# mit-han-lab/llm-awq

Hardware: AMD Instinct MI355X
Metric: W4A16 decode+prefill tok/s, Llama-3-8B; achieved %HBM (GEMV) / %MFMA (GEMM) (higher is better)
Workload: dtype bf16; 1 GPU; Llama-3-8B W4A16 g128 bf16 activations on 1xMI355X (decode GEMV + prefill GEMM); layers=32, decode_m=1, prefill_m=2048, graph=True, layout=cdna4, clock_ramp_steps=60, decode_mlp=gate/up + SiLU*mul launch, then down_proj, prefill_mlp=SiLU*mul fused into the gate/up GEMM epilogue, mlp=interleaved, decode_side_buffer=sz_half, parallelism=tp1, full=False

## Files before the change

llm_awq_amd/csrc/awq_gemm_plan.hip:

```cpp
#include <string.h>

#include <type_traits>

#include "awq_device.hpp"
#include "awq_kernels.hpp"

namespace awq {

namespace {
constexpr int TM = 256;
constexpr double kNarrowRate = 0.80;
int g_small_m = 1;
int g_splitk = 1;
int g_v6 = 1;
int g_tile_n = 0;
int g_v6_192 = 1;
int g_v6_pair = 1;
int g_v6_szh = 1;
int g_v4 = 1;
void launch_wide(const void* x, const void* qw, const void* szp, const void* bias, void* out, int m, int n, int k, int n_begin,
                 int n_end, int dtype, hipStream_t st, int bits, int epi, const void* szh = nullptr, int tile_n = 256) {
  if (g_v6 && m >= 256) {
    if (szh != nullptr && bits == 4 && g_v6_szh) launch_gemm_cdna4_v6(x, qw, szh, bias, out, m, n, k, n_begin, n_end, dtype, st, bits, epi, 1, tile_n);
    else launch_gemm_cdna4_v6(x, qw, szp, bias, out, m, n, k, n_begin, n_end, dtype, st, bits, epi, 0, tile_n);
    return;
  }
  launch_gemm_cdna4_v4n(x, qw, szp, bias, out, m, n, k, n_begin, n_end, dtype, nullptr, 0, st, bits, epi);
}
int g_v6_128 = 1;
int narrow_kernel(int m, int n_cols, int k, int bits, bool has_ws, int epi) {
  const size_t wsb = g_splitk && has_ws && epi == 0 ? gemm_v4n_workspace_bytes(m, n_cols, k) : 0;
  if (wsb > 0) return (int)(wsb / ((size_t)((m + TM - 1) / TM) * ((n_cols + 127) / 128) * TM * 128 * 4));
  return g_v6_128 && g_v6 && bits == 4 && m >= TM ? 1 : 0;
}
void launch_narrow(const void* x, const void* qw, const void* szp, const void* bias, void* out, int m, int n, int k, int n_begin,
                   int n_end, int dtype, void* ws, size_t ws_bytes, hipStream_t st, int bits, int epi, const void* szh = nullptr) {
  const bool use_szh = szh != nullptr && bits == 4 && g_v6_szh;
  if (g_v6 && g_v6_pair && g_splitk && !g_tile_n && ws != nullptr && m >= TM &&
      launch_gemm_cdna4_v6_pair(x, qw, use_szh ? szh : szp, bias, out, m, n, k, n_begin, n_end, dtype, ws, ws_bytes, st, bits, epi, use_szh ? 1 : 0) == 0)
    return;
  if (narrow_kernel(m, n_end - n_begin, k, bits, ws != nullptr, epi) == 1) {
    launch_gemm_cdna4_v6(x, qw, use_szh ? szh : szp, bias, out, m, n, k, n_begin, n_end, dtype, st, bits, epi, use_szh ? 1 : 0, 128);
    return;
  }
  launch_gemm_cdna4_v4n(x, qw, szp, bias, out, m, n, k, n_begin, n_end, dtype, g_splitk ? ws : nullptr, ws_bytes, st, bits, epi);
}
}

namespace {
int g_moe_v4 = 1;
}
bool moe_v4_enabled() { return g_moe_v4 != 0; }
namespace {
int g_moe_v6 = 1;
}
bool moe_v6_enabled() { return g_moe_v6 != 0; }

int gemm_v3_tune_set(const char* key, int value) {
  if (!strcmp(key, "moe_v6")) g_moe_v6 = value;
  else if (!strcmp(key, "moe_tail")) moe_v6_set_tail(value);
  else if (!strcmp(key, "gemm_v4")) g_v4 = value;
  else if (!strcmp(key, "gemm_v6")) {
    g_v6 = value % 10;
    gemm_v6_set_probe(value / 10);
  }
  else if (!strcmp(key, "gemm_tile_n")) g_tile_n = value;
  else if (!strcmp(key, "gemm_v6_szh")) g_v6_szh = value;
  else if (!strcmp(key, "gemm_v6_pair")) g_v6_pair = value;
  else if (!strcmp(key, "gemm_v6_pair_lead")) gemm_v6_set_pair_lead(value);
  else if (!strcmp(key, "gemm_v6_pair_min_nit")) gemm_v6_set_pair_min_nit(value);
  else if (!strcmp(key, "gemm_v6_192")) g_v6_192 = value;
  else if (!strcmp(key, "gemm_v6_128")) g_v6_128 = value;
  else if (!strcmp(key, "moe_v4")) g_moe_v4 = value;
  else if (!strcmp(key, "gemm_small_m")) g_small_m = value;
  else if (!strcmp(key, "gemm_splitk_cap")) g_v4n_ksplit_cap = value;
  else if (!strcmp(key, "gemm_splitk")) {
    g_splitk = value;
    g_v4n_ksplit_force = value > 1 ? value : 0;
  }
  else return -1;
  return 0;
}

namespace {
struct Plan {
  int mode;
  long cols_main;
};
constexpr double k192Rate = 0.97;
Plan plan_tiles(int m, int n, int tile_n, bool allow192 = false) {
  if (tile_n == 128) return {1, 0};
  if (tile_n == 256) return {0, 0};
  if (tile_n == 192) return {allow192 ? 3 : 0, 0};
  const long tiles_m = (m + TM - 1) / TM;
  auto rounds = [](long t) { return (double)((t + 255) / 256); };
  const long cols256 = (n + 255) / 256, t256 = tiles_m * cols256;
  const double cost_wide = rounds(t256);
  const double cost_narrow = rounds(tiles_m * ((n + 127) / 128)) * 0.5 / kNarrowRate;
  const long cols_main = (t256 / 256) * 256 / tiles_m;
  double cost_mixed = 1e30;
  if (cols_main > 0 && cols_main < cols256) {
    const long n_rest = n - cols_main * 256;
    cost_mixed = rounds(tiles_m * cols_main) + rounds(tiles_m * ((n_rest + 127) / 128)) * 0.5 / kNarrowRate + 0.02;
  }
  const double cost_192 = allow192 ? rounds(tiles_m * ((n + 191) / 192)) * 0.75 / k192Rate : 1e30;
  if (cost_192 < cost_wide && cost_192 < cost_narrow && cost_192 < cost_mixed) return {3, 0};
  if (cost_mixed < cost_wide && cost_mixed < cost_narrow) return {2, cols_main};
  return {cost_narrow < cost_wide ? 1 : 0, 0};
}
}

bool gemm_cdna4_v3_takes(int m, int k) {
  if (m >= TM) return true;
  if (g_small_m == 2) return g_v4 && m > 8;
  return g_small_m && g_v4 && m >= 72 && (long)m * k >= 600000;
}

size_t gemm_cdna4_v3_workspace_bytes(int m, int n, int k) {
  if (!gemm_cdna4_v3_takes(m, k) || (n % 16) != 0 || (k % 128) != 0 || !g_v4 || !g_splitk) return 0;
  if (gemm_cdna4_v3_pair_plan(m, n, k)) return gemm_v6_pair_workspace_bytes(m, n, k);
  if (m < TM) return gemm_v4n_workspace_bytes(m, n, k);
  const Plan p = plan_tiles(m, n, 0);
  if (p.mode == 1) return gemm_v4n_workspace_bytes(m, n, k);
  if (p.mode == 2) {
    const int rest = n - (int)(p.cols_main * 256);
    return gemm_cdna4_v3_pair_plan(m, rest, k) ? gemm_v6_pair_workspace_bytes(m, rest, k) : gemm_v4n_workspace_bytes(m, rest, k);
  }
  return 0;
}

int gemm_cdna4_v3_pair_plan(int m, int n, int k) { return g_v6 && g_v6_pair && g_splitk && !g_tile_n && gemm_v6_pair_takes(m, n, k) ? 1 : 0; }

size_t gemm_cdna4_v3_workspace_bytes_w3(int m, int n, int k) {
  if (m <= 8 || (n % 16) != 0 || (k % 128) != 0 || !g_splitk) return 0;
  if (gemm_cdna4_v3_pair_plan(m, n, k)) return gemm_v6_pair_workspace_bytes(m, n, k);
  if (m < TM) return gemm_v4n_workspace_bytes(m, n, k);
  const Plan p = plan_tiles(m, n, 0);
  if (p.mode == 1) return gemm_v4n_workspace_bytes(m, n, k);
  if (p.mode == 2) {
    const int rest = n - (int)(p.cols_main * 256);
    return gemm_cdna4_v3_pair_plan(m, rest, k) ? gemm_v6_pair_workspace_bytes(m, rest, k) : gemm_v4n_workspace_bytes(m, rest, k);
  }
  return 0;
}

int gemm_cdna4_v3_plan(int m, int n, int bits, int* mode, int* cols_main) {
  if (m <= 8 || (n % 16) != 0) return 0;
  const bool allow192 = g_v6 != 0 && g_v6_192 != 0 && bits == 4 && m >= TM;
  const Plan p = m < TM ? Plan{1, 0} : plan_tiles(m, n, g_tile_n, allow192);
  if (mode) *mode = p.mode;
  if (cols_main) *cols_main = (int)p.cols_main;
  const long tm = (m + TM - 1) / TM;
  if (p.mode == 0) return (int)(tm * ((n + 255) / 256));
  if (p.mode == 1) return (int)(tm * ((n + 127) / 128));
  if (p.mode == 3) return (int)(tm * ((n + 191) / 192));
  return (int)(tm * p.cols_main + tm * ((n - p.cols_main * 256 + 127) / 128));
}

// ... 30 lines not shown
```

llm_awq_amd/csrc/awq_gemm_v4n.hip:

```cpp
#include <type_traits>

#include "awq_device.hpp"
#include "awq_kernels.hpp"

namespace awq {

namespace {
constexpr int TM = 256, TN = 128, TK = 64;
constexpr int kTileX = TM * TK * 2;
constexpr int kTileW = TN * TK * 2;
constexpr int kWBase = 2 * kTileX;
constexpr int WN = 32;
typedef float f32x16 __attribute__((ext_vector_type(16)));

__device__ __forceinline__ int swz(int row) { return (row & 7) ^ ((row >> 4) & 1); }
__device__ __forceinline__ int tile_off(int row, int gc) { return row * 128 + ((gc ^ swz(row)) << 4); }

struct Group {
  u32x4 w;
  u32 b01, b23;
  float c;
};
struct Raw {
  u32x4 w;
  u32 sz;
};
template <int V>
using ic = std::integral_constant<int, V>;
template <bool V>
using bc = std::integral_constant<bool, V>;
template <int WIDX, int ST>
struct JobT {
  static constexpr bool has = true;
  static constexpr int widx = WIDX, st = ST;
};
struct NoJob {
  static constexpr bool has = false;
  static constexpr int widx = 0, st = 0;
};
}

#define V4N_READ(dst, addr, off) asm volatile("ds_read_b128 %0, %1 offset:%2" : "=v"(dst) : "v"(addr), "n"(off) : "memory")
#define V4N_WRITE(addr, val, off) asm volatile("ds_write_b128 %0, %1 offset:%2\n\ts_nop 1" : : "v"(addr), "v"(val), "n"(off) : "memory")
#define V4N_FENCE() __builtin_amdgcn_sched_barrier(0)

template <typename DT, int KSPLIT, int PARTIAL, int BITS = 4>
__global__ __launch_bounds__(512) void gemm_cdna4_v4n_kernel(const uint16_t* __restrict__ x, const u32* __restrict__ qw,
                                                             const u32* __restrict__ szp, const uint16_t* __restrict__ bias,
                                                             uint16_t* __restrict__ out, int M, int N, int K, int tiles_m,
                                                             int tiles_n, int n_begin, int n_end, int ksplit,
                                                             float* __restrict__ partial, int epi) {
  using vec8 = typename DT::vec8;
  constexpr int kEpiRow = 2 * WN + 16;
  extern __shared__ __attribute__((aligned(16))) char smem[];
  const int tid = threadIdx.x, lane = tid & 63, wv = tid >> 6;
  const int i = lane & 15, g = lane >> 4;
  const int l32 = lane & 31, hk = lane >> 5;
  const int wm = wv >> 2, wn = wv & 3;

  const int T = tiles_m * tiles_n;
  const int split = KSPLIT ? (int)(blockIdx.x % (unsigned)ksplit) : 0;
  int tile;
  {
    const int b = KSPLIT ? (int)(blockIdx.x / (unsigned)ksplit) : (int)blockIdx.x, xcd = b & 7, idx = b >> 3;
    const int q = T >> 3, r = T & 7;
    tile = (xcd < r ? xcd * (q + 1) : r * (q + 1) + (xcd - r) * q) + idx;
  }
  int tm, tn;
  {
    const int full = (tiles_m >> 1) * 2 * tiles_n;
    if (tile < full) {
      const int band = tile / (2 * tiles_n), rem = tile - band * 2 * tiles_n;
      tn = rem >> 1;
      tm = 2 * band + (rem & 1);
    } else {
      tn = tile - full;
      tm = tiles_m - 1;
    }
  }
  const int m0 = max(min(tm * TM, M - TM), 0), n0 = n_begin + tn * TN;
  const int nit_all = K >> 7;
  const int g0 = KSPLIT ? split * nit_all / ksplit : 0;
  const int nit = KSPLIT ? (split + 1) * nit_all / ksplit - g0 : nit_all;

  u32 a_off[4];
  {
    const int row = tid >> 3, gcp = tid & 7;
    const int gc = gcp ^ swz(row);
#pragma unroll
    for (int q = 0; q < 4; ++q) a_off[q] = (u32)min(m0 + row + 64 * q, M - 1) * (u32)K + gc * 8;
  }
  const int a_rows = PARTIAL ? M - m0 - (tid >> 3) : 256;
  auto issue_a = [&](int kt, int stage) {
    char* dst = smem + stage * kTileX + wv * 1024;
#pragma unroll
    for (int q = 0; q < 4; ++q) {
      const uint16_t* xq = x + (size_t)(kt + 2 * g0) * TK;
      if (!PARTIAL || 64 * q < a_rows)
        __builtin_amdgcn_global_load_lds((const __attribute__((address_space(1))) void*)(xq + a_off[q]),
                                       (__attribute__((address_space(3))) void*)(dst + q * 8192), 16, 0, 0);
    }
  };

  const int nslab = N >> 4;
  const int sl = min((n0 >> 4) + wv, min(nslab, n_end >> 4) - 1);
  constexpr int kTileWords = BITS == 4 ? 256 : 192, kLaneWords = BITS == 4 ? 4 : 3;
  const u32 b_off = (u32)sl * nit_all * kTileWords + lane * kLaneWords, sz_off = (u32)sl * nit_all * 16 + i;
  const int nl = 16 * wv + i;
  Cdna4DequantT<DT> cd;
  cd.init(lane, BITS == 4 ? 0x000F000Fu : 0x00070007u);
  auto load_group = [&](int grp) {
    Raw r;
    const u32* wp = qw + (size_t)(g0 + grp) * kTileWords + b_off;
    if (BITS == 4) {
      r.w = *reinterpret_cast<const u32x4*>(wp);
    } else {
      typedef u32 u32x3 __attribute__((ext_vector_type(3)));
      const u32x3 w3 = *reinterpret_cast<const u32x3*>(wp);
      r.w = u32x4{w3.x, w3.y, w3.z, 0u};
    }
    r.sz = szp[(size_t)(g0 + grp) * 16 + sz_off];
    return r;
  };
  auto prep = [&](const Raw& r) {
    Group gq;
    gq.w = BITS == 4 ? r.w : w3_expand(r.w.x, r.w.y, r.w.z);
    const u32 sd = (r.sz & 0xFFFFu) * 0x00010001u;
    gq.b01 = sd & cd.m01;
    gq.b23 = sd & cd.m23;
    gq.c = DT::dq_offset(r.sz);
    return gq;
  };

  const u32 lds0 = (u32)(size_t)(__attribute__((address_space(3))) char*)smem;
// ... 64 lines not shown
      asm volatile("s_waitcnt lgkmcnt(3)" : "+v"(wc), "+v"(x0));
      mfb(ic<0>{}, wc, x0);
      V4N_FENCE();
      asm volatile("s_waitcnt lgkmcnt(2)" : "+v"(x1));
      mfb(ic<1>{}, wc, x1);
      V4N_FENCE();
      asm volatile("s_waitcnt lgkmcnt(0)" : "+v"(x2), "+v"(x3));
      __syncthreads();
      V4N_FENCE();
      if constexpr (J::has) {
        const vec8 v = Cdna4DequantT<DT>::word_finish(pj);
        V4N_WRITE(ja[J::widx & 1], __builtin_bit_cast(u32x4, v), J::st * kTileW);
      }
      if constexpr (RD) {
        V4N_READ(wnx, wa[KN], SN * kTileW);
        V4N_READ(x0, xa[KN], SN * kTileX);
        V4N_READ(x1, xa[KN], SN * kTileX + 4096);
      }
      V4N_FENCE();
      mfb(ic<2>{}, wc, x2);
      V4N_FENCE();
      if constexpr (RD) V4N_READ(x2, xa[KN], SN * kTileX + 8192);
      mfb(ic<3>{}, wc, x3);
      V4N_FENCE();
      if constexpr (RD) V4N_READ(x3, xa[KN], SN * kTileX + 12288);
      V4N_FENCE();
    }
  };

  issue_a(0, 0);
  gc = prep(load_group(0));
  Raw rn = load_group(nit > 1 ? 1 : 0);
  {
    char* Bs = smem + kWBase;
    *reinterpret_cast<vec8*>(Bs + tile_off(nl, 0 + g)) = cd.word(gc.w.x, gc.b01, gc.b23, gc.c);
    *reinterpret_cast<vec8*>(Bs + tile_off(nl, 4 + g)) = cd.word(gc.w.y, gc.b01, gc.b23, gc.c);
  }
  __syncthreads();
  asm volatile("" : "+v"(rn.w), "+v"(rn.sz));
  issue_a(1, 1);
  V4N_FENCE();
  {
    const vec8 v = cd.word(gc.w.z, gc.b01, gc.b23, gc.c);
    V4N_WRITE(ja[0], __builtin_bit_cast(u32x4, v), kTileW);
  }
  V4N_READ(wf[0], wa[0], 0);
  V4N_READ(x0, xa[0], 0);
  V4N_READ(x1, xa[0], 4096);
  V4N_READ(x2, xa[0], 8192);
  V4N_READ(x3, xa[0], 12288);
  V4N_FENCE();

  auto group_iter = [&](int q, auto more_tag) {
    constexpr bool more = decltype(more_tag)::value;
    using Tt = bc<true>;
    using Ff = bc<false>;
    step(ic<0>{}, ic<0>{}, ic<1>{}, Tt{}, Ff{}, NoJob{});
    step(ic<1>{}, ic<0>{}, ic<2>{}, Tt{}, Ff{}, JobT<3, 1>{});
    step(ic<0>{}, ic<0>{}, ic<3>{}, Tt{}, Ff{}, NoJob{});
    if constexpr (more) {
      gc = prep(rn);
      step(ic<1>{}, ic<1>{}, ic<0>{}, Tt{}, Tt{}, JobT<0, 0>{});
      rn = load_group(min(q + 2, nit - 1));
      issue_a(2 * q + 2, 0);
      V4N_FENCE();
      step(ic<0>{}, ic<1>{}, ic<1>{}, Tt{}, Ff{}, NoJob{});
      step(ic<1>{}, ic<1>{}, ic<2>{}, Tt{}, Ff{}, JobT<1, 0>{});
      step(ic<0>{}, ic<1>{}, ic<3>{}, Tt{}, Ff{}, NoJob{});
      step(ic<1>{}, ic<0>{}, ic<0>{}, Tt{}, Tt{}, JobT<2, 1>{});
      issue_a(2 * q + 3, 1);
      V4N_FENCE();
    } else {
      step(ic<1>{}, ic<1>{}, ic<0>{}, Tt{}, Tt{}, NoJob{});
      step(ic<0>{}, ic<1>{}, ic<1>{}, Tt{}, Ff{}, NoJob{});
      step(ic<1>{}, ic<1>{}, ic<2>{}, Tt{}, Ff{}, NoJob{});
      step(ic<0>{}, ic<1>{}, ic<3>{}, Tt{}, Ff{}, NoJob{});
      step(ic<1>{}, ic<0>{}, ic<0>{}, Ff{}, Tt{}, NoJob{});
    }
  };
  for (int q = 0; q + 1 < nit; ++q) group_iter(q, std::true_type{});
  group_iter(nit - 1, std::false_type{});

  if constexpr (KSPLIT != 0) {
    float* base = partial + (((size_t)tile * ksplit + split) * 8 + wv) * (4 * 4 * 64 * 4);
#pragma unroll
    for (int b = 0; b < 4; ++b)
#pragma unroll
      for (int j = 0; j < 4; ++j)
        *reinterpret_cast<f32x4*>(base + ((b * 4 + j) * 64 + lane) * 4) =
            f32x4{acc[b][4 * j + 0], acc[b][4 * j + 1], acc[b][4 * j + 2], acc[b][4 * j + 3]};
    return;
  }
  if (epi == 3) {
    float* o32 = reinterpret_cast<float*>(out);
#pragma unroll
    for (int b = 0; b < 4; ++b) {
      const int m = m0 + wm * 128 + b * 32 + l32;
#pragma unroll
      for (int j = 0; j < 4; ++j) {
        const int nn = n0 + wn * WN + 8 * j + 4 * hk;
        if (nn < n_end && m < M)
          __builtin_nontemporal_store(f32x4{acc[b][4 * j + 0], acc[b][4 * j + 1], acc[b][4 * j + 2], acc[b][4 * j + 3]}, reinterpret_cast<f32x4*>(o32 + (size_t)m * N + nn));
      }
    }
    return;
  }
  __syncthreads();
  char* eb = smem + wv * (128 * kEpiRow);
#pragma unroll
  for (int b = 0; b < 4; ++b)
#pragma unroll
    for (int j = 0; j < 4; ++j) {
      u32x2 v;
      v.x = (u32)DT::from_float(acc[b][4 * j + 0]) | ((u32)DT::from_float(acc[b][4 * j + 1]) << 16);
      v.y = (u32)DT::from_float(acc[b][4 * j + 2]) | ((u32)DT::from_float(acc[b][4 * j + 3]) << 16);
      *reinterpret_cast<u32x2*>(eb + (b * 32 + l32) * kEpiRow + (8 * j + 4 * hk) * 2) = v;
    }
  __builtin_amdgcn_s_waitcnt(0xc07f);
  __builtin_amdgcn_wave_barrier();
  constexpr int GR = WN / 8, RP = 64 / GR;
#pragma unroll
  for (int ps = 0; ps < 128 / RP; ++ps) {
    const int row = ps * RP + lane / GR, gc2 = lane % GR;
    const int m = m0 + wm * 128 + row, nn = n0 + wn * WN + gc2 * 8;
    u32x4 v = *reinterpret_cast<const u32x4*>(eb + row * kEpiRow + gc2 * 16);
    if (epi == 2) {
      if ((gc2 & 1) == 0 && nn < n_end && m < M) {
        const u32x4 u = *reinterpret_cast<const u32x4*>(eb + row * kEpiRow + (gc2 + 1) * 16);
        __builtin_nontemporal_store(silu_mul_octet<DT>(v, u), reinterpret_cast<u32x4*>(out + (size_t)m * (N >> 1) + (nn >> 1)));
      }
      continue;
    }
    if (nn < n_end && m < M) {
      if (bias != nullptr) {
        const u32x4 bv = *reinterpret_cast<const u32x4*>(bias + nn);
        auto add2 = [](u32 a, u32 b) {
          const float lo = DT::to_float((uint16_t)(a & 0xFFFFu)) + DT::to_float((uint16_t)(b & 0xFFFFu));
          const float hi = DT::to_float((uint16_t)(a >> 16)) + DT::to_float((uint16_t)(b >> 16));
          return (u32)DT::from_float(lo) | ((u32)DT::from_float(hi) << 16);
        };
        v = u32x4{add2(v.x, bv.x), add2(v.y, bv.y), add2(v.z, bv.z), add2(v.w, bv.w)};
      }
      __builtin_nontemporal_store(v, reinterpret_cast<u32x4*>(out + (size_t)m * N + nn));
    }
  }
}

template <typename DT>
__global__ __launch_bounds__(256) void splitk_reduce_kernel(const float* __restrict__ partial, const uint16_t* __restrict__ bias,
                                                            uint16_t* __restrict__ out, int M, int N, int tiles_m, int tiles_n,
                                                            int n_begin, int n_end, int ksplit) {
  constexpr int kRow = 2 * WN + 16;
  __shared__ __attribute__((aligned(16))) char stage[4][32 * kRow];
  const int lane = threadIdx.x & 63, w = threadIdx.x >> 6;
  const int piece = blockIdx.x * 4 + w;
  const int b = piece & 3, wv = (piece >> 2) & 7, tile = piece >> 5;
  if (tile >= tiles_m * tiles_n) return;
  const int l32 = lane & 31, hk = lane >> 5, wm = wv >> 2, wn = wv & 3;
  int tm, tn;
  {
    const int full = (tiles_m >> 1) * 2 * tiles_n;
    if (tile < full) {
      const int band = tile / (2 * tiles_n), rem = tile - band * 2 * tiles_n;
      tn = rem >> 1;
      tm = 2 * band + (rem & 1);
    } else {
      tn = tile - full;
      tm = tiles_m - 1;
    }
  }
  constexpr size_t kWaveFloats = 4 * 4 * 64 * 4;
  const float* p = partial + (((size_t)tile * ksplit) * 8 + wv) * kWaveFloats + ((size_t)(b * 4) * 64 + lane) * 4;
  f32x4 acc[4];
#pragma unroll
  for (int j = 0; j < 4; ++j) acc[j] = f32x4{0.f, 0.f, 0.f, 0.f};
  for (int s2 = 0; s2 < ksplit; ++s2) {
    f32x4 v[4];
#pragma unroll
    for (int j = 0; j < 4; ++j) v[j] = *reinterpret_cast<const f32x4*>(p + (size_t)s2 * 8 * kWaveFloats + j * 256);
#pragma unroll
    for (int j = 0; j < 4; ++j) acc[j] += v[j];
  }
  char* eb = stage[w];
#pragma unroll
  for (int j = 0; j < 4; ++j) {
    u32x2 v;
    v.x = (u32)DT::from_float(acc[j][0]) | ((u32)DT::from_float(acc[j][1]) << 16);
    v.y = (u32)DT::from_float(acc[j][2]) | ((u32)DT::from_float(acc[j][3]) << 16);
    *reinterpret_cast<u32x2*>(eb + l32 * kRow + (8 * j + 4 * hk) * 2) = v;
  }
  __builtin_amdgcn_s_waitcnt(0xc07f);
  __builtin_amdgcn_wave_barrier();
  const int m_base = max(min(tm * TM, M - TM), 0) + wm * 128 + b * 32, n_base = n_begin + tn * TN + wn * WN;
#pragma unroll
  for (int ps = 0; ps < 2; ++ps) {
    const int row = ps * 16 + (lane >> 2), gc2 = lane & 3;
    const int nn = n_base + gc2 * 8;
    u32x4 v = *reinterpret_cast<const u32x4*>(eb + row * kRow + gc2 * 16);
    if (nn < n_end && m_base + row < M) {
      if (bias != nullptr) {
        const u32x4 bv = *reinterpret_cast<const u32x4*>(bias + nn);
        auto add2 = [](u32 a, u32 c) {
          const float lo = DT::to_float((uint16_t)(a & 0xFFFFu)) + DT::to_float((uint16_t)(c & 0xFFFFu));
          const float hi = DT::to_float((uint16_t)(a >> 16)) + DT::to_float((uint16_t)(c >> 16));
          return (u32)DT::from_float(lo) | ((u32)DT::from_float(hi) << 16);
        };
        v = u32x4{add2(v.x, bv.x), add2(v.y, bv.y), add2(v.z, bv.z), add2(v.w, bv.w)};
      }
      *reinterpret_cast<u32x4*>(out + (size_t)(m_base + row) * N + nn) = v;
    }
  }
}

int g_v4n_ksplit_cap = 1;
int g_v4n_ksplit_force = 0;
int gemm_v4n_ksplit(int m, int n_cols, int k) {
  const long tiles = (long)((m + TM - 1) / TM) * ((n_cols + TN - 1) / TN);
  const int nit = k / 128;
  if (g_v4n_ksplit_force > 1) return g_v4n_ksplit_force <= nit && tiles * g_v4n_ksplit_force <= 1024 ? g_v4n_ksplit_force : 1;
  auto rounds = [](long blocks) { return (double)((blocks + 255) / 256); };
  const double unsplit = rounds(tiles) * (nit + 2.0);
  double best_cost = 0.9 * unsplit;
  int best = 1;
  for (int d = 2; d <= 16 && nit / d >= 2; ++d) {
    if (g_v4n_ksplit_cap && tiles * d > 192 && tiles * d <= 256 && nit / d <= 8) continue;
    const double cost = rounds(tiles * d) * ((nit + d - 1) / d + 0.6) + 0.041 * (double)(tiles * d) + 1.3;
    if (cost < best_cost) {
      best_cost = cost;
      best = d;
    }
  }
  return best;
}
size_t gemm_v4n_workspace_bytes(int m, int n_cols, int k) {
  const int ks = gemm_v4n_ksplit(m, n_cols, k);
  if (ks <= 1) return 0;
  const size_t tiles = (size_t)((m + TM - 1) / TM) * ((n_cols + TN - 1) / TN);
  return tiles * ks * (size_t)TM * TN * 4;
}

void launch_gemm_cdna4_v4n(const void* x, const void* qw, const void* szp, const void* bias, void* out, int m, int n, int k,
                           int n_begin, int n_end, int dtype, void* ws, size_t ws_bytes, hipStream_t st, int bits, int epi) {
  constexpr int smem_main = 2 * kTileX + 2 * kTileW;
  constexpr int smem_epi = 8 * 128 * (2 * WN + 16);
  constexpr int smem = smem_main > smem_epi ? smem_main : smem_epi;
  const int tiles_m = (m + TM - 1) / TM, tiles_n = (n_end - n_begin + TN - 1) / TN;
  using Kern = void (*)(const uint16_t*, const u32*, const u32*, const uint16_t*, uint16_t*, int, int, int, int, int, int, int, int, float*, int);
  static const Kern kerns4[2][2][2] = {
      {{gemm_cdna4_v4n_kernel<F16, 0, 0>, gemm_cdna4_v4n_kernel<F16, 0, 1>}, {gemm_cdna4_v4n_kernel<F16, 1, 0>, gemm_cdna4_v4n_kernel<F16, 1, 1>}},
      {{gemm_cdna4_v4n_kernel<BF16, 0, 0>, gemm_cdna4_v4n_kernel<BF16, 0, 1>}, {gemm_cdna4_v4n_kernel<BF16, 1, 0>, gemm_cdna4_v4n_kernel<BF16, 1, 1>}}};
  static const Kern kerns3[2][2][2] = {
      {{gemm_cdna4_v4n_kernel<F16, 0, 0, 3>, gemm_cdna4_v4n_kernel<F16, 0, 1, 3>}, {gemm_cdna4_v4n_kernel<F16, 1, 0, 3>, gemm_cdna4_v4n_kernel<F16, 1, 1, 3>}},
      {{gemm_cdna4_v4n_kernel<BF16, 0, 0, 3>, gemm_cdna4_v4n_kernel<BF16, 0, 1, 3>}, {gemm_cdna4_v4n_kernel<BF16, 1, 0, 3>, gemm_cdna4_v4n_kernel<BF16, 1, 1, 3>}}};
  const Kern (*kerns)[2][2] = bits == 3 ? kerns3 : kerns4;
  static LdsOptIn optin[2][8];
  for (int a = 0; a < 8; ++a) optin[bits == 3][a].ensure(reinterpret_cast<const void*>(kerns[a >> 2][(a >> 1) & 1][a & 1]), smem);
  const int dt = dtype == 0 ? 0 : 1, partial = m <= TM - 32 ? 1 : 0;
  const int ks = gemm_v4n_ksplit(m, n_end - n_begin, k);
  const size_t need = ks > 1 ? (size_t)tiles_m * tiles_n * ks * TM * TN * 4 : 0;
  if (epi == 0 && ks > 1 && ws != nullptr && ws_bytes >= need && (reinterpret_cast<uintptr_t>(ws) & 15) == 0) {
    hipLaunchKernelGGL(kerns[dt][1][partial], dim3(tiles_m * tiles_n * ks), dim3(512), smem, st, (const uint16_t*)x, (const u32*)qw,
                       (const u32*)szp, (const uint16_t*)nullptr, (uint16_t*)out, m, n, k, tiles_m, tiles_n, n_begin, n_end, ks, (float*)ws, 0);
    auto red = dtype == 0 ? splitk_reduce_kernel<F16> : splitk_reduce_kernel<BF16>;
    hipLaunchKernelGGL(red, dim3((unsigned)(tiles_m * tiles_n * 8)), dim3(256), 0, st, (const float*)ws, (const uint16_t*)bias, (uint16_t*)out,
                       m, n, tiles_m, tiles_n, n_begin, n_end, ks);
    return;
  }
  hipLaunchKernelGGL(kerns[dt][0][partial], dim3(tiles_m * tiles_n), dim3(512), smem, st, (const uint16_t*)x, (const u32*)qw,
                     (const u32*)szp, (const uint16_t*)bias, (uint16_t*)out, m, n, k, tiles_m, tiles_n, n_begin, n_end, 1, (float*)nullptr, epi);
}

}
```

llm_awq_amd/csrc/awq_kernels.hpp:

```cpp
#pragma once
#include <hip/hip_runtime.h>
#include <stddef.h>
#include <stdint.h>

#include <atomic>

namespace awq {
struct LdsOptIn {
  std::atomic<uint64_t> done[4] = {};
  void ensure(const void* kern, int bytes = 160 * 1024) {
    int dev = 0;
    (void)hipGetDevice(&dev);
    const uint64_t bit = 1ull << (dev & 63);
    std::atomic<uint64_t>& w = done[(dev >> 6) & 3];
    if (w.load(std::memory_order_acquire) & bit) return;
    (void)hipFuncSetAttribute(kern, hipFuncAttributeMaxDynamicSharedMemorySize, bytes);
    w.fetch_or(bit, std::memory_order_release);
  }
};
inline int device_cu_count() {
  static std::atomic<int> cached[64] = {};
  int dev = 0;
  if (hipGetDevice(&dev) != hipSuccess) return 256;
  std::atomic<int>& c = cached[dev & 63];
  int v = c.load(std::memory_order_relaxed);
  if (v == 0) {
    if (hipDeviceGetAttribute(&v, hipDeviceAttributeMultiprocessorCount, dev) != hipSuccess || v <= 0) v = 256;
    c.store(v, std::memory_order_relaxed);
  }
  return v;
}
int launch_gemv(const void* x, const void* qw, const void* s, const void* z, const void* szp, void* out, int m, int n,
                int k, int dtype, int layout, hipStream_t st);
int launch_gemv_cdna4(const void* x, const void* qw, const void* szp, const void* bias, void* out, int m, int n, int k,
                      int epi, int bits, int dtype, hipStream_t st);
int launch_gemv_cdna4_norm(const void* x, const void* gamma, float eps, const void* qw, const void* szp, const void* bias, void* out,
                           int m, int n, int k, int epi, int dtype, hipStream_t st);
bool gemv_v2fast_enabled();
int launch_gemv_v2fast(const void* x, const void* qw, const void* s, const void* z, const void* bias, void* out, int m, int n, int k,
                       int gpad, int dtype, hipStream_t st);
int launch_skinny_v2(const void* x, const void* qw, const void* s, const void* z, const void* bias, void* out, int m, int n, int k,
                     int gpad, int dtype, hipStream_t st);
int launch_pack_w3(const void* q_u8, void* qw3, int n, int k, hipStream_t st);
int launch_unpack_w3(const void* qw3, void* out_u8, int n, int k, hipStream_t st);
int launch_dequant_w3(const void* qw3, const void* s, const void* z, void* out, int n, int k, int dtype, hipStream_t st);
int launch_expand_w3_to_cdna4(const void* qw3, void* qw4, int n, int k, hipStream_t st);
int gemv_cdna4_tune_set(const char* key, int value);
int launch_gemv_dma(const void* x, const void* qw, const void* szp, const void* bias, void* out, int m, int n, int k, int epi,
                    int dtype, int szfmt, hipStream_t st, int f32out = 0);
int gemv_dma_tune_set(const char* key, int value);
int launch_moe_gemv_cdna4(const void* x, const void* qw, const void* szp, const void* offsets, void* out, int total_rows,
                          int experts, int n, int k, int dtype, hipStream_t st);
int launch_moe_skinny_tail_cdna4(const void* x, const void* qw, const void* szp, const void* offsets, void* out, int experts, int n, int k,
                                 int dtype, hipStream_t st, int epi, int tail);
void moe_v6_set_tail(int v);
int launch_moe_skinny_cdna4(const void* x, const void* qw, const void* szp, const void* offsets, void* out, int total_rows,
                            int experts, int n, int k, int dtype, hipStream_t st);
int launch_pack_sz_cdna4(const void* s, const void* z, void* szp, int n, int k, hipStream_t st);
int launch_pack_szh_cdna4(const void* s, const void* z, void* szh, int* inexact, int n, int k, int dtype, hipStream_t st);
int launch_gemm(const void* x, const void* qw, const void* s, const void* z, const void* szp, void* out, int m, int n,
                int k, int dtype, int layout, void* ws, size_t ws_bytes, hipStream_t st);
int launch_repack_v2_cdna4(const void* src, void* dst, int n, int k, int to_cdna4, hipStream_t st);
int launch_unpack_cdna4(const void* qw, void* out_u8, int n, int k, hipStream_t st);
int launch_dequant_cdna4(const void* qw, const void* s, const void* z, void* out, int n, int k, int dtype, hipStream_t st);
size_t gemm_workspace_bytes(int m, int n, int k);
int launch_gemm_cdna4_v3(const void* x, const void* qw, const void* szp, const void* bias, void* out, int m, int n, int k,
                         int tile_n, int dtype, void* ws, size_t ws_bytes, hipStream_t st, int bits = 4, int epi = 0, const void* szh = nullptr);
int gemm_variant_get();
int launch_skinny_cdna4(const void* x, const void* qw, const void* szp, const void* bias, void* out, int m, int n, int k,
                        int dtype, hipStream_t st, int f32out = 0, void* ws = nullptr, size_t ws_bytes = 0);
int launch_skinny_w3(const void* x, const void* qw, const void* szp, const void* bias, void* out, int m, int n, int k, int epi, int dtype, hipStream_t st,
                     int f32out = 0);
int launch_skinny_gate_up(const void* x, const void* qw, const void* szp, void* out, int m, int n2, int k, int dtype, hipStream_t st);
int skinny_splitk_parts(int m, int n, int k);
size_t skinny_splitk_workspace_bytes(int m, int n, int k);
int skinny_tune_set(const char* key, int value);
int launch_midm_cdna4(const void* x, const void* qw, const void* szp, const void* bias, void* out, int m, int n, int k, int epi, int dtype, int szfmt,
                      int bits, int f32out, void* ws, size_t ws_bytes, hipStream_t st);
bool midm_takes(int m, int n, int k);
size_t midm_workspace_bytes(int m, int n, int k);
int midm_parts(int m, int n, int k);
int midm_tune_set(const char* key, int value);
int midm_init();
unsigned* splitk_ticket_words(hipStream_t st, int groups);
int launch_skinny_decode(const void* x, const void* qw, const void* szp, const void* bias, void* out, int m, int n, int k, int epi,
                         int dtype, int szfmt, hipStream_t st, int f32out = 0);
int launch_moe_gemm(const void* x, const void* qw, const void* s, const void* z, const void* offsets, void* out, int total_m,
                    int experts, int n, int k, int gpad, int dtype, int layout, hipStream_t st);
int gemv_tune_set(const char* key, int value);
int gemm_tune_set(const char* key, int value);
int gemm_v3_tune_set(const char* key, int value);
void launch_gemm_cdna4_v4n(const void* x, const void* qw, const void* szp, const void* bias, void* out, int m, int n, int k,
                           int n_begin, int n_end, int dtype, void* ws, size_t ws_bytes, hipStream_t st, int bits = 4, int epi = 0);
size_t gemm_v4n_workspace_bytes(int m, int n_cols, int k);
extern int g_v4n_ksplit_force;
extern int g_v4n_ksplit_cap;
bool gemm_cdna4_v3_takes(int m, int k);
size_t gemm_cdna4_v3_workspace_bytes(int m, int n, int k);
int gemm_cdna4_v3_plan(int m, int n, int bits, int* mode, int* cols_main);
int gemm_cdna4_v3_narrow_kernel(int m, int n_cols, int k, int bits, int has_workspace, int epi);
int gemv_dma_plan(int m, int n, int k, int epi, int* kernel);
size_t gemm_cdna4_v3_workspace_bytes_w3(int m, int n, int k);
bool moe_v4_enabled();
int launch_moe_gemm_cdna4_v6(const void* x, const void* qw, const void* szp, const void* offsets, void* out, int total, int experts,
                             int n, int k, int dtype, hipStream_t st, int epi = 0, const void* szh = nullptr);
int launch_silu_mul_interleaved(const void* in, void* out, int m, int n2, int dtype, hipStream_t st);
int launch_silu_mul(const void* gate, const void* up, void* out, size_t count, int dtype, hipStream_t st);
bool moe_v6_enabled();
void launch_gemm_cdna4_v6(const void* x, const void* qw, const void* szp, const void* bias, void* out, int m, int n, int k, int n_begin,
                          int n_end, int dtype, hipStream_t st, int bits = 4, int epi = 0, int szfmt = 0, int tile_n = 256);
void gemm_v6_set_probe(int v);
bool gemm_v6_pair_takes(int m, int n, int k);
int gemm_v6_pair_lost(unsigned* count);
int gemm_cdna4_v3_pair_plan(int m, int n, int k);
size_t gemm_v6_pair_workspace_bytes(int m, int n, int k);
int launch_gemm_cdna4_v6_pair(const void* x, const void* qw, const void* szp, const void* bias, void* out, int m, int n, int k, int n_begin, int n_end,
                              int dtype, void* ws, size_t ws_bytes, hipStream_t st, int bits = 4, int epi = 0, int szfmt = 0);
void gemm_v6_set_pair_lead(int v);
void gemm_v6_set_pair_min_nit(int v);
int launch_bias_add(void* out, const void* bias, int m, int n, int dtype, hipStream_t st);
int launch_round_bias_f32(const void* in_f32, const void* bias, void* out, int m, int n, int dtype, hipStream_t st);
int launch_rmsnorm(const void* x, const void* gamma, float eps, void* out, int m, int k, int dtype, hipStream_t st);
int attn_decode_plan(int batch, int nheads_kv, int head_dim, int timestep, int lmax, int* splits, int* chunk);
size_t attn_decode_workspace_bytes(int batch, int nheads, int nheads_kv, int head_dim, int timestep, int lmax);
int launch_attn_decode(const void* q, const void* k, const void* v, void* k_cache, void* v_cache, const int* lens, const float* alibi,
                       void* out, int B, int H, int Hkv, int Dh, int Lmax, long long q_bs, long long k_bs, long long v_bs, int timestep,
                       int rot, float rot_base, float rot_scale, int neox, int dtype, void* workspace, hipStream_t st);
int attn_prefill_plan(int batch, int nheads, int nheads_kv, int head_dim, int seqlen_q, int seqlen_k, int causal, int* q_tile_rows,
                      int* blocks);
int attn_prefill_tune_set(const char* key, int value);
int launch_attn_prefill(const void* q, const void* k, const void* v, void* out, int B, int Sq, int Sk, int H, int Hkv, int Dh, long long q_bs,
                        long long q_rs, long long k_bs, long long k_rs, long long v_bs, long long v_rs, float scale, int causal, int dtype,
                        hipStream_t st);
int launch_rope_with_pos(const void* in, const float* freqs, void* out, int n0, int n1, int h, int d, int d2, long long s0, long long s1,
                         long long sh, long long o0, long long o1, long long oh, int dtype, hipStream_t st);
int launch_rope_neox(const long long* positions, void* query, void* key, const void* cache, int tokens, int heads, int head_size, int rot_dim,
                     int max_pos, int dtype, hipStream_t st);
int w8a8_gemm_plan(int m, int n, int k, int* tile_m, int* tile_n);
int w8a8_tune_set(const char* key, int value);
int launch_w8a8_gemm(const void* x, const void* w, const void* wscales, const void* ascales, const void* bias, void* out, int m, int n, int k,
                     hipStream_t st);
int launch_quant_per_token(const void* x, void* out_i8, void* scale, int m, int k, int dtype, hipStream_t st);
int launch_gelu_quant_per_token(const void* x, void* out_i8, void* scale, void* tmp, int m, int k, hipStream_t st);
int launch_layernorm_quant(const void* x, const void* gamma, const void* beta, float eps, void* out_i8, void* scale, int m, int k,
                           int per_token, int dtype, hipStream_t st);
int launch_unpack_v2(const void* qw, void* out_u8, int n, int k, hipStream_t st);
int launch_dequant_v2(const void* qw, const void* s, const void* z, void* out, int n, int k, int dtype, hipStream_t st);
int launch_pack_v2(const void* q_u8, void* qw, int n, int k, hipStream_t st);
int launch_repack_v1_to_v2(const void* qw1, const void* s1, const void* qz1, void* qw2, void* s2, void* sz2, int n, int k,
                           int gpad, int dtype, hipStream_t st);
}
```

llm_awq_amd/csrc/awq_midm_cdna4.hip:

```cpp
#include <string.h>

#include <atomic>
#include <mutex>
#include <type_traits>

#include "awq_device.hpp"
#include "awq_dma.hpp"
#include "awq_kernels.hpp"

#ifdef AWQ_ENABLE_PROBES
__device__ unsigned long long g_midm_stamps[2048 * 8];
extern "C" __attribute__((visibility("default"))) int awq_dev_midm_stamps(void* host_dst, int blocks) {
  return (int)hipMemcpyFromSymbol(host_dst, HIP_SYMBOL(g_midm_stamps), (size_t)blocks * 64, 0, hipMemcpyDeviceToHost);
}
#define MIDM_STAMP(j)                                                                \
  if (threadIdx.x == 0 && blockIdx.y == 0 && blockIdx.x < 2048) {                    \
    g_midm_stamps[blockIdx.x * 8 + 2 * (j)] = __builtin_amdgcn_s_memrealtime();      \
    g_midm_stamps[blockIdx.x * 8 + 2 * (j) + 1] = __builtin_readcyclecounter();      \
  }
#else
#define MIDM_STAMP(j)
#endif

namespace awq {

namespace {
constexpr u32 kOob = 0x80000000u;
}

template <int C, int CB>
__device__ __forceinline__ void midm_read_x(u32x4 (&dst)[CB], u32 addr) {
  if constexpr (C < CB) {
    asm volatile("ds_read_b128 %0, %1 offset:%2" : "=v"(dst[C]) : "v"(addr), "n"(C * 4096) : "memory");
    midm_read_x<C + 1, CB>(dst, addr);
  }
}

template <int S>
__device__ __forceinline__ void midm_read_w(u32x4& w, u32& sz, u32 waddr, u32 saddr) {
  asm volatile("ds_read_b128 %0, %1 offset:%2" : "=v"(w) : "v"(waddr), "n"(S * 1280) : "memory");
  asm volatile("ds_read_b32 %0, %1 offset:%2" : "=v"(sz) : "v"(saddr), "n"(S * 1280) : "memory");
}

template <typename DT, int THREADS, int NSB>
__device__ __forceinline__ void midm_reduce_parts(char* smem, const float* __restrict__ parts, u32* __restrict__ tickets, const uint16_t* __restrict__ bias,
                                                  uint16_t* __restrict__ out, int M, int N, int KS, int nb, int epi, int f32out) {
  const int nslab = N >> 4;
  auto to_f = [](uint16_t b) { return DT::to_float(b); };
  asm volatile("s_waitcnt vmcnt(0)" : : : "memory");
  __syncthreads();
  u32* bc = reinterpret_cast<u32*>(smem);
  if (threadIdx.x == 0) bc[0] = __hip_atomic_fetch_add(tickets + nb, 1u, __ATOMIC_RELAXED, __HIP_MEMORY_SCOPE_AGENT);
  __syncthreads();
  if (bc[0] != (u32)(KS - 1)) return;
  if (threadIdx.x == 0) __hip_atomic_store(tickets + nb, 0u, __ATOMIC_RELAXED, __HIP_MEMORY_SCOPE_AGENT);
  const int col0 = nb * NSB * 16;
  auto sum_quad = [&](int m, int col) {
    f32x4 a = f32x4{0.f, 0.f, 0.f, 0.f};
    for (int p0 = 0; p0 < KS; p0 += 4) {
      f32x4 v[4];
#pragma unroll
      for (int j = 0; j < 4; ++j) {
        const float* src = parts + ((size_t)min(p0 + j, KS - 1) * M + m) * N + col;
        asm volatile("global_load_dwordx4 %0, %1, off sc1" : "=v"(v[j]) : "v"(src) : "memory");
      }
      asm volatile("s_waitcnt vmcnt(0)" : "+v"(v[0]), "+v"(v[1]), "+v"(v[2]), "+v"(v[3]) : : "memory");
#pragma unroll
      for (int j = 0; j < 4; ++j)
        if (p0 + j < KS) a += v[j];
    }
    return a;
  };
  if (epi == 2) {
    constexpr int QC = NSB * 2;
    for (int idx = threadIdx.x; idx < M * QC; idx += THREADS) {
      const int m = idx / QC, q = idx - m * QC, sl = q >> 1, h = q & 1;
      const int slab = nb * NSB + sl;
      if (slab >= nslab) continue;
      const f32x4 gt4 = sum_quad(m, col0 + sl * 16 + 4 * h), up4 = sum_quad(m, col0 + sl * 16 + 8 + 4 * h);
      uint16_t o[4];
#pragma unroll
      for (int r = 0; r < 4; ++r) {
        const float gt = to_f(DT::from_float(gt4[r])), u = to_f(DT::from_float(up4[r]));
        const float sl2 = to_f(DT::from_float(silu_f32(gt)));
        o[r] = DT::from_float(sl2 * u);
      }
      *reinterpret_cast<u32x2*>(out + (size_t)m * (N >> 1) + slab * 8 + 4 * h) = u32x2{(u32)o[0] | ((u32)o[1] << 16), (u32)o[2] | ((u32)o[3] << 16)};
// ... 230 lines not shown
              if (bias != nullptr) o[r] = DT::from_float(to_f(o[r]) + to_f(bias[nn + r]));
            }
            *reinterpret_cast<u32x2*>(out + (size_t)m * N + nn) = u32x2{(u32)o[0] | ((u32)o[1] << 16), (u32)o[2] | ((u32)o[3] << 16)};
          }
        }
      }
    }
#ifdef AWQ_ENABLE_PROBES
    asm volatile("s_waitcnt vmcnt(0)" ::: "memory");
#endif
    MIDM_STAMP(3)
    return;
  }

  {
    float* mine = parts + (size_t)p * M * N;
#pragma unroll
    for (int s = 0; s < NS; ++s) {
      const int slab = nb * NSB + wv * NS + s;
#pragma unroll
      for (int c = 0; c < CB; ++c) {
        const int m = 16 * c + i;
        if (slab < nslab && m < M) {
          float* dst = mine + (size_t)m * N + slab * 16 + 4 * g;
          asm volatile("global_store_dwordx4 %0, %1, off sc1\n\ts_nop 1" : : "v"(dst), "v"(acc[s][c]) : "memory");
        }
      }
    }
  }
  midm_reduce_parts<DT, 64 * WAVES, NSB>(smem, parts, tickets, bias, out, M, N, KS, nb, epi, f32out);
}

namespace {
constexpr int kStreamLanes = 64, kLaneWords = 1024;
constexpr int kCaptureWords = 1 << 20;
struct TicketPool {
  u32* base = nullptr;
  hipStream_t lane_stream[kStreamLanes] = {};
  bool lane_used[kStreamLanes] = {};
  int capture_next = 0;
};
std::mutex g_ticket_mu;
TicketPool g_pools[64];
}


unsigned* splitk_ticket_words(hipStream_t st, int groups) {
  int dev = 0;
  if (st == hipStreamPerThread) return nullptr;
  if (groups > kLaneWords || hipGetDevice(&dev) != hipSuccess || dev < 0 || dev >= 64) return nullptr;
  hipStreamCaptureStatus cs = hipStreamCaptureStatusNone;
  if (st != nullptr && hipStreamIsCapturing(st, &cs) != hipSuccess) return nullptr;
  const bool capturing = cs != hipStreamCaptureStatusNone;
  std::lock_guard<std::mutex> lock(g_ticket_mu);
  TicketPool& tp = g_pools[dev];
  if (tp.base == nullptr) {
    if (capturing) return nullptr;
    u32* fresh = nullptr;
    const size_t bytes = ((size_t)kStreamLanes * kLaneWords + kCaptureWords) * sizeof(u32);
    if (hipMalloc(reinterpret_cast<void**>(&fresh), bytes) != hipSuccess) return nullptr;
    if (hipMemset(fresh, 0, bytes) != hipSuccess || hipStreamSynchronize(nullptr) != hipSuccess) {
      (void)hipFree(fresh);
      return nullptr;
    }
    tp.base = fresh;
  }
  if (capturing) {
    if (tp.capture_next + groups > kCaptureWords) return nullptr;
    u32* w = tp.base + (size_t)kStreamLanes * kLaneWords + tp.capture_next;
    tp.capture_next += groups;
    return w;
  }
  int free_lane = -1;
  for (int l = 0; l < kStreamLanes; ++l) {
    if (tp.lane_used[l] && tp.lane_stream[l] == st) return tp.base + (size_t)l * kLaneWords;
    if (!tp.lane_used[l] && free_lane < 0) free_lane = l;
  }
  if (free_lane < 0) return nullptr;
  tp.lane_used[free_lane] = true;
  tp.lane_stream[free_lane] = st;
  return tp.base + (size_t)free_lane * kLaneWords;
}

namespace {

int g_midm = 1;
int g_midm_min = 65, g_midm_max = 128;
int g_midm_waves = 0, g_midm_ns = 0, g_midm_ks = 0;
int g_midm_probe = 0;
}

int midm_tune_set(const char* key, int value) {
  if (!strcmp(key, "midm")) g_midm = value;
  else if (!strcmp(key, "midm_min")) g_midm_min = value;
  else if (!strcmp(key, "midm_max")) g_midm_max = value;
  else if (!strcmp(key, "midm_waves")) g_midm_waves = value;
  else if (!strcmp(key, "midm_ns")) g_midm_ns = value;
  else if (!strcmp(key, "midm_ks")) g_midm_ks = value;
  else if (!strcmp(key, "midm_probe")) g_midm_probe = value;
  else return -1;
  return 0;
}

namespace {
struct MidmCfg {
  int waves, ns, cb, ks;
};
constexpr int midm_xstage(int cb, int waves) { return (4 * cb + waves - 1) / waves * waves * 1024; }
constexpr int midm_lds(int cb, int waves, int ns, int dx) { return dx * midm_xstage(cb, waves) + waves * ns * (dx + 1) * 1280; }
constexpr int midm_dx(int cb, int waves, int ns) {
  int dx = 8;
  while (dx > 3 && midm_lds(cb, waves, ns, dx) > 150 * 1024) --dx;
  return dx;
}
int ks_for(int groups, int nit, int cus) {
  int ks = 1;
  while (groups * ks * 2 <= cus && nit / (ks * 2) >= 2) ks *= 2;
  return ks;
}
bool midm_pick(int m, int n, int k, bool may_split, MidmCfg& c) {
  const int nslab = n / 16, nit = k / 128, cus = device_cu_count();
  c.cb = (m + 15) / 16;
  c.ns = g_midm_ns ? g_midm_ns : 1;
  if (g_midm_waves) c.waves = g_midm_waves;
  else {
    const int g8 = (nslab + 8 * c.ns - 1) / (8 * c.ns);
    c.waves = nit / ks_for(g8, nit, cus) >= 8 ? 8 : 4;
  }
  const int groups = (nslab + c.waves * c.ns - 1) / (c.waves * c.ns);
  int ks = g_midm_ks > 0 ? g_midm_ks : ks_for(groups, nit, cus);
  if (ks > nit / 2) ks = nit / 2 > 0 ? nit / 2 : 1;
  if (!may_split || ks < 1) ks = 1;
  c.ks = ks;
  return c.cb >= 1 && c.cb <= 8 && ((c.waves == 8 && c.ns == 1) || (c.waves == 4 && (c.ns == 1 || c.ns == 2))) &&
         midm_lds(c.cb, c.waves, c.ns, midm_dx(c.cb, c.waves, c.ns)) <= 160 * 1024;
}
void midm_passes(int m, int& chunks, int& rows) {
  chunks = (m + 127) / 128;
  rows = (m + chunks - 1) / chunks;
}
}

namespace {
bool midm_small_takes(int m, int n, int k) {
  const int nslab = n / 16, nit = k / 128, cus = device_cu_count();
  const int g7 = (nslab + 6) / 7;
  const bool seven_round = g7 <= cus + 16 && g7 >= cus * 9 / 10;
  if (m >= 17 && m <= 32 && n >= 16384) return true;
  if (nit >= 192 && nslab <= 512) return true;
  if (m >= 33 && nslab >= 512 && nslab < 640) return true;
  if (m >= 49 && n >= 16384 && !seven_round) return true;
  return false;
}
}
bool midm_takes(int m, int n, int k) {
  if (!g_midm || m < 9 || m > 255 || (n % 16) != 0 || (k % 128) != 0 || k < 256) return false;
  if (g_midm_min == 65 && g_midm_max == 128) {
    if (m > 128 || (m < 65 && !midm_small_takes(m, n, k))) return false;
  } else {
    if (m < g_midm_min || m > g_midm_max) return false;
    if (m > 128 && n >= 16384 && g_midm_max <= 192) return false;
  }
  if ((size_t)n * (size_t)k / 2 >= (1ull << 31) || (size_t)m * (size_t)k * 2 >= (1ull << 31)) return false;
  int chunks, rows;
  midm_passes(m, chunks, rows);
  MidmCfg c;
// ... 86 lines not shown
```

Baseline: 1008 decode tok/s (the 160 quantised linears of one token: 32 x {qkv, o, gate, up, down}; attention/norm/lm_head off-path).

## Fuse split-K reduction into v4n GEMM via per-tile ticket counters

Adds a last-block-reduces path to the split-K v4n GEMM. Each split writes its fp32 partials with sc1 stores, then atomically bumps a per-tile ticket, and the block that arrives last sums all partials in a software-pipelined load loop and runs the normal epilogue. This removes the separate splitk_reduce kernel launch and its extra pass over the workspace. It is enabled by default for small tile counts and low split factors through a heuristic. The cost is atomics, cache-coherence store flags, extra register pressure in the tail, and reset bookkeeping for the tickets.

```diff
diff --git a/llm_awq_amd/csrc/awq_gemm_plan.hip b/llm_awq_amd/csrc/awq_gemm_plan.hip
--- a/llm_awq_amd/csrc/awq_gemm_plan.hip
+++ b/llm_awq_amd/csrc/awq_gemm_plan.hip
@@ -74,6 +74,7 @@
   else if (!strcmp(key, "moe_v4")) g_moe_v4 = value;
   else if (!strcmp(key, "gemm_small_m")) g_small_m = value;
   else if (!strcmp(key, "gemm_splitk_cap")) g_v4n_ksplit_cap = value;
+  else if (!strcmp(key, "gemm_splitk_fused")) g_v4n_fused = value;
   else if (!strcmp(key, "gemm_splitk")) {
     g_splitk = value;
     g_v4n_ksplit_force = value > 1 ? value : 0;
diff --git a/llm_awq_amd/csrc/awq_gemm_v4n.hip b/llm_awq_amd/csrc/awq_gemm_v4n.hip
--- a/llm_awq_amd/csrc/awq_gemm_v4n.hip
+++ b/llm_awq_amd/csrc/awq_gemm_v4n.hip
@@ -49,7 +49,7 @@
                                                              const u32* __restrict__ szp, const uint16_t* __restrict__ bias,
                                                              uint16_t* __restrict__ out, int M, int N, int K, int tiles_m,
                                                              int tiles_n, int n_begin, int n_end, int ksplit,
-                                                             float* __restrict__ partial, int epi) {
+                                                             float* __restrict__ partial, int epi, u32* __restrict__ tickets) {
   using vec8 = typename DT::vec8;
   constexpr int kEpiRow = 2 * WN + 16;
   extern __shared__ __attribute__((aligned(16))) char smem[];
@@ -280,16 +280,77 @@
   group_iter(nit - 1, std::false_type{});
 
   if constexpr (KSPLIT != 0) {
-    float* base = partial + (((size_t)tile * ksplit + split) * 8 + wv) * (4 * 4 * 64 * 4);
+    constexpr size_t kWaveFloats = 4 * 4 * 64 * 4;
+    float* base = partial + (((size_t)tile * ksplit + split) * 8 + wv) * kWaveFloats + lane * 4;
+    if (tickets == nullptr) {
+#pragma unroll
+      for (int b = 0; b < 4; ++b)
+#pragma unroll
+        for (int j = 0; j < 4; ++j)
+          *reinterpret_cast<f32x4*>(base + (b * 4 + j) * 256) = f32x4{acc[b][4 * j + 0], acc[b][4 * j + 1], acc[b][4 * j + 2], acc[b][4 * j + 3]};
+      return;
+    }
 #pragma unroll
     for (int b = 0; b < 4; ++b)
 #pragma unroll
-      for (int j = 0; j < 4; ++j)
-        *reinterpret_cast<f32x4*>(base + ((b * 4 + j) * 64 + lane) * 4) =
-            f32x4{acc[b][4 * j + 0], acc[b][4 * j + 1], acc[b][4 * j + 2], acc[b][4 * j + 3]};
-    return;
-  }
-  if (epi == 3) {
+      for (int j = 0; j < 4; ++j) {
+        const f32x4 v = f32x4{acc[b][4 * j + 0], acc[b][4 * j + 1], acc[b][4 * j + 2], acc[b][4 * j + 3]};
+        const float* dst = base + (b * 4 + j) * 256;
+        asm volatile("global_store_dwordx4 %0, %1, off sc1\n\ts_nop 1" : : "v"(dst), "v"(v) : "memory");
+      }
+    asm volatile("s_waitcnt vmcnt(0)" : : : "memory");
+    __syncthreads();
+    u32* bcast = reinterpret_cast<u32*>(smem + 8 * 128 * kEpiRow);
+    if (tid == 0) bcast[0] = __hip_atomic_fetch_add(tickets + tile, 1u, __ATOMIC_RELAXED, __HIP_MEMORY_SCOPE_AGENT);
+    __syncthreads();
+    if (bcast[0] != (u32)(ksplit - 1)) return;
+    const float* part0 = partial + ((size_t)tile * ksplit * 8 + wv) * kWaveFloats + lane * 4;
+    f32x16 sum[4];
+#pragma unroll
+    for (int b = 0; b < 4; ++b)
+#pragma unroll
+      for (int r = 0; r < 16; ++r) sum[b][r] = 0.f;
+    auto issue = [&](f32x4(&v)[8], int s, int h) {
+      const float* src = part0 + (size_t)s * (8 * kWaveFloats) + h * 2048;
+#pragma unroll
+      for (int q = 0; q < 8; ++q) asm volatile("global_load_dwordx4 %0, %1, off sc1" : "=v"(v[q]) : "v"(src + q * 256) : "memory");
+    };
+    auto add_half = [&](int h, const f32x4(&v)[8]) {
+#pragma unroll
+      for (int q = 0; q < 8; ++q)
+#pragma unroll
+        for (int r = 0; r < 4; ++r) sum[2 * h + (q >> 2)][4 * (q & 3) + r] += v[q][r];
+    };
+#define V4N_LANDED(cnt, v)                                                                                                                      \
+  asm volatile("s_waitcnt vmcnt(" #cnt ")" : "+v"(v[0]), "+v"(v[1]), "+v"(v[2]), "+v"(v[3]), "+v"(v[4]), "+v"(v[5]), "+v"(v[6]), "+v"(v[7]) : : "memory")
+    auto add_ranges = [&](int lo, int hi) {
+      if (lo >= hi) return;
+      f32x4 va[8], vb[8];
+      issue(va, lo, 0);
+      for (int s = lo; s + 1 < hi; ++s) {
+        issue(vb, s, 1);
+        V4N_LANDED(8, va);
+        add_half(0, va);
+        issue(va, s + 1, 0);
+        V4N_LANDED(8, vb);
+        add_half(1, vb);
+      }
+      issue(vb, hi - 1, 1);
+      V4N_LANDED(8, va);
+      add_half(0, va);
+      V4N_LANDED(0, vb);
+      add_half(1, vb);
+    };
+    add_ranges(0, split);
+#pragma unroll
+    for (int b = 0; b < 4; ++b) sum[b] += acc[b];
+    add_ranges(split + 1, ksplit);
+#undef V4N_LANDED
+    if (tid == 0) __hip_atomic_store(tickets + tile, 0u, __ATOMIC_RELAXED, __HIP_MEMORY_SCOPE_AGENT);
+#pragma unroll
+    for (int b = 0; b < 4; ++b) acc[b] = sum[b];
+  }
+  if (KSPLIT == 0 && epi == 3) {
     float* o32 = reinterpret_cast<float*>(out);
 #pragma unroll
     for (int b = 0; b < 4; ++b) {
@@ -412,6 +473,12 @@
 
 int g_v4n_ksplit_cap = 1;
 int g_v4n_ksplit_force = 0;
+int g_v4n_fused = 1;
+static bool v4n_fused_pays(long tiles, int nit, int ks) { return tiles * ks <= 256 && (ks <= 3 || (ks == 4 && nit / ks <= 8)); }
+namespace {
+std::atomic<unsigned> g_v4n_fused_launches{0};
+}
+extern "C" __attribute__((visibility("default"))) unsigned awq_dev_v4n_fused_launches(void) { return g_v4n_fused_launches.load(std::memory_order_relaxed); }
 int gemm_v4n_ksplit(int m, int n_cols, int k) {
   const long tiles = (long)((m + TM - 1) / TM) * ((n_cols + TN - 1) / TN);
   const int nit = k / 128;
@@ -443,7 +510,7 @@
   constexpr int smem_epi = 8 * 128 * (2 * WN + 16);
   constexpr int smem = smem_main > smem_epi ? smem_main : smem_epi;
   const int tiles_m = (m + TM - 1) / TM, tiles_n = (n_end - n_begin + TN - 1) / TN;
-  using Kern = void (*)(const uint16_t*, const u32*, const u32*, const uint16_t*, uint16_t*, int, int, int, int, int, int, int, int, float*, int);
+  using Kern = void (*)(const uint16_t*, const u32*, const u32*, const uint16_t*, uint16_t*, int, int, int, int, int, int, int, int, float*, int, u32*);
   static const Kern kerns4[2][2][2] = {
       {{gemm_cdna4_v4n_kernel<F16, 0, 0>, gemm_cdna4_v4n_kernel<F16, 0, 1>}, {gemm_cdna4_v4n_kernel<F16, 1, 0>, gemm_cdna4_v4n_kernel<F16, 1, 1>}},
       {{gemm_cdna4_v4n_kernel<BF16, 0, 0>, gemm_cdna4_v4n_kernel<BF16, 0, 1>}, {gemm_cdna4_v4n_kernel<BF16, 1, 0>, gemm_cdna4_v4n_kernel<BF16, 1, 1>}}};
@@ -457,15 +524,21 @@
   const int ks = gemm_v4n_ksplit(m, n_end - n_begin, k);
   const size_t need = ks > 1 ? (size_t)tiles_m * tiles_n * ks * TM * TN * 4 : 0;
   if (epi == 0 && ks > 1 && ws != nullptr && ws_bytes >= need && (reinterpret_cast<uintptr_t>(ws) & 15) == 0) {
+    const bool fused = g_v4n_fused >= 2 || (g_v4n_fused == 1 && v4n_fused_pays((long)tiles_m * tiles_n, k / 128, ks));
+    u32* tk = fused ? splitk_ticket_words(st, tiles_m * tiles_n) : nullptr;
     hipLaunchKernelGGL(kerns[dt][1][partial], dim3(tiles_m * tiles_n * ks), dim3(512), smem, st, (const uint16_t*)x, (const u32*)qw,
-                       (const u32*)szp, (const uint16_t*)nullptr, (uint16_t*)out, m, n, k, tiles_m, tiles_n, n_begin, n_end, ks, (float*)ws, 0);
+                       (const u32*)szp, (const uint16_t*)(tk ? bias : nullptr), (uint16_t*)out, m, n, k, tiles_m, tiles_n, n_begin, n_end, ks, (float*)ws, 0, tk);
+    if (tk != nullptr) {
+      g_v4n_fused_launches.fetch_add(1, std::memory_order_relaxed);
+      return;
+    }
     auto red = dtype == 0 ? splitk_reduce_kernel<F16> : splitk_reduce_kernel<BF16>;
     hipLaunchKernelGGL(red, dim3((unsigned)(tiles_m * tiles_n * 8)), dim3(256), 0, st, (const float*)ws, (const uint16_t*)bias, (uint16_t*)out,
                        m, n, tiles_m, tiles_n, n_begin, n_end, ks);
     return;
   }
   hipLaunchKernelGGL(kerns[dt][0][partial], dim3(tiles_m * tiles_n), dim3(512), smem, st, (const uint16_t*)x, (const u32*)qw,
-                     (const u32*)szp, (const uint16_t*)bias, (uint16_t*)out, m, n, k, tiles_m, tiles_n, n_begin, n_end, 1, (float*)nullptr, epi);
-}
-
-}
+                     (const u32*)szp, (const uint16_t*)bias, (uint16_t*)out, m, n, k, tiles_m, tiles_n, n_begin, n_end, 1, (float*)nullptr, epi, (u32*)nullptr);
+}
+
+}
diff --git a/llm_awq_amd/csrc/awq_kernels.hpp b/llm_awq_amd/csrc/awq_kernels.hpp
--- a/llm_awq_amd/csrc/awq_kernels.hpp
+++ b/llm_awq_amd/csrc/awq_kernels.hpp
@@ -95,6 +95,7 @@
 size_t gemm_v4n_workspace_bytes(int m, int n_cols, int k);
 extern int g_v4n_ksplit_force;
 extern int g_v4n_ksplit_cap;
+extern int g_v4n_fused;
 bool gemm_cdna4_v3_takes(int m, int k);
 size_t gemm_cdna4_v3_workspace_bytes(int m, int n, int k);
 int gemm_cdna4_v3_plan(int m, int n, int bits, int* mode, int* cols_main);
diff --git a/llm_awq_amd/csrc/awq_midm_cdna4.hip b/llm_awq_amd/csrc/awq_midm_cdna4.hip
--- a/llm_awq_amd/csrc/awq_midm_cdna4.hip
+++ b/llm_awq_amd/csrc/awq_midm_cdna4.hip
@@ -3,6 +3,7 @@
 #include <atomic>
 #include <mutex>
 #include <type_traits>
+#include <vector>
 
 #include "awq_device.hpp"
 #include "awq_dma.hpp"
@@ -399,6 +400,20 @@
   return tp.base + (size_t)free_lane * kLaneWords;
 }
 
+extern "C" __attribute__((visibility("default"))) int awq_dev_splitk_tickets_nonzero(void) {
+  int dev = 0;
+  if (hipGetDevice(&dev) != hipSuccess || dev < 0 || dev >= 64 || hipDeviceSynchronize() != hipSuccess) return -1;
+  std::lock_guard<std::mutex> lock(g_ticket_mu);
+  const TicketPool& tp = g_pools[dev];
+  if (tp.base == nullptr) return -1;
+  const size_t words = (size_t)kStreamLanes * kLaneWords + (size_t)tp.capture_next;
+  std::vector<u32> host(words);
+  if (hipMemcpy(host.data(), tp.base, words * sizeof(u32), hipMemcpyDeviceToHost) != hipSuccess) return -1;
+  int busy = 0;
+  for (u32 w : host) busy += w != 0;
+  return busy;
+}
+
 namespace {
 
 int g_midm = 1;
```

New measurement: 1002 decode tok/s (the 160 quantised linears of one token: 32 x {qkv, o, gate, up, down}; attention/norm/lm_head off-path). Within noise of the previous version (-0.6%).
